# microsoft/tutel

Measured on NVIDIA H100. Metric: moe_layer_fwd_bwd_tokens_per_sec, higher is better.
Workload: dtype bf16; 1 GPU; model=helloworld moe_layer top-2 8-expert ffn(relu) model_dim=4096 hidden=14336, global_batch=16, seq_len=512, parallelism=ep1 (8 local experts/GPU), a2a_ffn_overlap_degree=1, cuda_graph=True, launches_per_graph_replay=15

## Files before the change

### csrc/gemm_sm90.cu

```cuda
#include "gemm_sm90.h"

#include <cuda.h>
#include <cuda_bf16.h>
#include <cuda_fp16.h>

#include <cstdio>
#include <cstdlib>
#include <mutex>

#include "ptx.cuh"

namespace tb {

struct GemmArgs {
  int M, N, K, G;
  int b_group_div;
  int tiles_m, tiles_n;
  long long num_tiles;

  void* d;
  long long ldd, d_group_stride;
  const unsigned long long* d_ptr_table;
  int out_dtype;

// ... 30 lines not shown
namespace {

constexpr int kThreads = 384;
constexpr int kSwizzleBytes = 128;
constexpr int kSmemLimit = 232448;

template <int BN_>
struct Cfg {
  static constexpr int BM = 128;
  static constexpr int BN = BN_;
  static constexpr bool WIDE = BN_ == 256;
  static constexpr int A_BYTES = BM * kSwizzleBytes;
  static constexpr int B_BYTES = BN * kSwizzleBytes;
  static constexpr int STAGE_BYTES = A_BYTES + B_BYTES;
  static constexpr int EPI_COLS = 128;
  static constexpr int PASSES = BN / EPI_COLS;
  static constexpr int EPI_PITCH = EPI_COLS + 8;
  static constexpr int EPI_WARP_BYTES = 16 * EPI_PITCH * 4;
  static constexpr int EPI_BYTES = 8 * EPI_WARP_BYTES;
  static constexpr int BAR_BYTES = 512;
  static constexpr int STAGES = WIDE ? 3 : 4;
  static constexpr int MAXNREG = WIDE ? 168 : 144;
  static constexpr int CONSUMER_REGS = WIDE ? 232 : 192;
  static constexpr int SMEM_BYTES = STAGES * STAGE_BYTES + 1024 + BAR_BYTES + EPI_BYTES;
  static_assert(WIDE || SMEM_BYTES + 2 * 1024 <= 228 * 1024, "no room for the push kernel");
  static_assert(SMEM_BYTES <= kSmemLimit, "");
  static_assert(128 * 40 + 256 * CONSUMER_REGS <= 65536 && 384 * MAXNREG <= 65536, "register budget");
};

struct TileCoord {
  int g, m_blk, n_blk;
};

template <int kBand>
__device__ __forceinline__ TileCoord decode_tile(long long t, int tiles_m, int tiles_n) {
  const int per_group = tiles_m * tiles_n;
  TileCoord c;
  c.g = static_cast<int>(t / per_group);
  int r = static_cast<int>(t - static_cast<long long>(c.g) * per_group);
// ... 10 lines not shown
__device__ __forceinline__ int rotate_group(int g, int rot, int mod) {
  if (mod > 1) {
    const int base = (g / mod) * mod;
    return base + (g - base + rot) % mod;
  }
  if (mod < -1) {
    const int m = -mod;
    const int base = (g / m) * m;
    return base + (rot + m - (g - base)) % m;
  }
  return g;
}

__device__ __forceinline__ float gelu_erf(float x) { return 0.5f * x * (1.0f + erff(x * 0.70710678118654752f)); }
__device__ __forceinline__ float silu(float x) { return __fdividef(x, 1.0f + __expf(-x)); }

__device__ __forceinline__ void unpack8(const uint4& u, bool is_bf16, float* f) {
  const uint32_t w[4] = {u.x, u.y, u.z, u.w};
#pragma unroll
  for (int i = 0; i < 4; ++i) {
    if (is_bf16) {
      f[2 * i] = __uint_as_float(w[i] << 16);
      f[2 * i + 1] = __uint_as_float(w[i] & 0xFFFF0000u);
    } else {
      const __half2 h = *reinterpret_cast<const __half2*>(&w[i]);
      const float2 t = __half22float2(h);
      f[2 * i] = t.x;
      f[2 * i + 1] = t.y;
    }
  }
// ... 23 lines not shown
    for (int i = 0; i < 4; ++i) {
      if constexpr (BF16) {
        f[q * 8 + 2 * i] = __uint_as_float(w[i] << 16);
        f[q * 8 + 2 * i + 1] = __uint_as_float(w[i] & 0xFFFF0000u);
      } else {
        const float2 t = __half22float2(*reinterpret_cast<const __half2*>(&w[i]));
        f[q * 8 + 2 * i] = t.x;
        f[q * 8 + 2 * i + 1] = t.y;
      }
    }
  }
}
__device__ __forceinline__ void unpack32(const uint4* p, float* f, bool is_bf16) {
  if (is_bf16) unpack32_t<true>(p, f); else unpack32_t<false>(p, f);
}

__device__ __forceinline__ float fast_sigmoid(float x) { return __fdividef(1.0f, 1.0f + __expf(-x)); }

template <int ACT>
__device__ __forceinline__ void glu_fwd_seg(const float* g, const float* u, float* o) {
#pragma unroll
  for (int j = 0; j < 32; ++j) {
    float a;
    if constexpr (ACT == ACT_RELU) a = fmaxf(g[j], 0.0f);
    else if constexpr (ACT == ACT_GELU) a = gelu_erf(g[j]);
    else a = g[j] * fast_sigmoid(g[j]);
    o[j] = a * u[j];
  }
}
template <int ACT>
__device__ __forceinline__ void glu_bwd_seg(const float* r, const float* g, float* u, float* o) {
#pragma unroll
// ... 5 lines not shown
      da = g[j] > 0.0f ? 1.0f : 0.0f;
    } else if constexpr (ACT == ACT_GELU) {
      const float cdf = 0.5f * (1.0f + erff(g[j] * 0.70710678118654752f));
      a = g[j] * cdf;
      da = cdf + g[j] * 0.3989422804014327f * __expf(-0.5f * g[j] * g[j]);
    } else {
      const float sg = fast_sigmoid(g[j]);
      a = g[j] * sg;
      da = sg * (1.0f + g[j] * (1.0f - sg));
    }
    o[j] = dh * u[j] * da;
    u[j] = dh * a;
  }
}

template <int BN_, bool A_MN, bool B_MN, int DT>
__global__ void __maxnreg__(Cfg<BN_>::MAXNREG)
gemm_sm90_kernel(const __grid_constant__ CUtensorMap tmA, const __grid_constant__ CUtensorMap tmB,
                 const __grid_constant__ CUtensorMap tmB2, const GemmArgs args) {
  using C = Cfg<BN_>;
  constexpr int BN = C::BN;
  extern __shared__ uint8_t smem_raw[];

  const int warp = __shfl_sync(0xffffffffu, static_cast<int>(threadIdx.x >> 5), 0);
  const int lane = threadIdx.x & 31;

  const uint32_t smem_base = (ptx::smem_u32(smem_raw) + 1023u) & ~1023u;
  constexpr int stages = C::STAGES;
  const uint32_t bar_base = smem_base + static_cast<uint32_t>(stages) * C::STAGE_BYTES;
  auto smem_a = [&](int s) { return smem_base + s * C::STAGE_BYTES; };
  auto smem_b = [&](int s) { return smem_base + s * C::STAGE_BYTES + C::A_BYTES; };
  auto full_bar = [&](int s) { return bar_base + 8u * s; };
  auto empty_bar = [&](int s) { return bar_base + 64u + 8u * s; };
  const uint32_t epi_base = bar_base + C::BAR_BYTES;
  float* epi_ptr = reinterpret_cast<float*>(smem_raw + (epi_base - ptx::smem_u32(smem_raw)));

  if (warp == 0 && ptx::elect_one()) {
    ptx::prefetch_tensormap(&tmA);
    ptx::prefetch_tensormap(&tmB);
    if (args.dual) ptx::prefetch_tensormap(&tmB2);
  }
  if (warp == 1 && lane == 0) {
    for (int s = 0; s < stages; ++s) {
      ptx::mbar_init(full_bar(s), 1);
      ptx::mbar_init(empty_bar(s), 2);
    }
    ptx::fence_mbar_init();
  }
  __syncthreads();

  constexpr int kEltBytes = (DT == DT_E4M3 || DT == DT_E5M2) ? 1 : 2;
  static_assert(kEltBytes == 2 || (!A_MN && !B_MN), "8-bit operands are K-major only");
  const int num_kb = (args.K * kEltBytes + kSwizzleBytes - 1) / kSwizzleBytes;
  constexpr int bk_elems = kSwizzleBytes / kEltBytes;
  const long long tile_step = gridDim.x;
  const long long tile_first = blockIdx.x;
  constexpr int kBand = 16;
  const bool dual = !C::WIDE && args.dual != 0;
  const int tile_n = dual ? BN / 2 : BN;

  if (warp < 4) {
    ptx::setmaxnreg_dec<40>();
    if (warp == 0) {
      int s = 0;
      uint32_t ph = 0;
      int seen_group = -1;
      unsigned long long seen_mask = 0ull;
      for (long long t = tile_first; t < args.num_tiles; t += tile_step) {
        TileCoord tc = decode_tile<kBand>(t, args.tiles_m, args.tiles_n);
        tc.g = rotate_group(tc.g, args.group_rot, args.group_mod);
        if (args.row_counts != nullptr && tc.m_blk * C::BM >= args.row_counts[tc.g]) continue;
        const int m0 = tc.m_blk * C::BM;
        const int n0 = tc.n_blk * BN;
        const int gb = tc.g / args.b_group_div;
        if (args.wait_flags != nullptr) {
          if (tc.g != seen_group) { seen_group = tc.g; seen_mask = 0ull; }
          const int f0 = (tc.m_blk * C::BM) / args.wait_rows_per_flag;
          const int f1 = (min(tc.m_blk * C::BM + C::BM, args.M) - 1) / args.wait_rows_per_flag;
          unsigned long long need = 0ull;
          for (int f = f0; f <= f1; ++f) need |= 1ull << (f & 63);
// ... 33 lines not shown
            } else {
              const int nb0 = tc.n_blk * (BN / 2);
              if constexpr (!B_MN) {
                ptx::tma_load_3d(smem_b(s), &tmB, fb, k0, nb0, gb);
                ptx::tma_load_3d(smem_b(s) + (BN / 2) * kSwizzleBytes, &tmB2, fb, k0, nb0, gb);
              } else {
                constexpr int half_chunks = (BN / 2) / chunk_elems;
                for (int c = 0; c < 2 * half_chunks; ++c)
                  ptx::tma_load_3d(smem_b(s) + c * chunk_bytes, c < half_chunks ? &tmB : &tmB2, fb,
                                   nb0 + (c % half_chunks) * chunk_elems, k0, gb);
              }
            }
          }
          __syncwarp();
          if (++s == stages) { s = 0; ph ^= 1u; }
        }
      }
    }
  } else {
    ptx::setmaxnreg_inc<C::CONSUMER_REGS>();
    const int cw = warp - 4;
    const int wg = cw >> 2;
    const bool wg_leader = (threadIdx.x & 127) == 0;
    int s = 0;
    uint32_t ph = 0;
    constexpr uint32_t kMnChunkBytes = 64u * kSwizzleBytes;
    constexpr uint32_t kMnKStep = 16u * kSwizzleBytes;
    constexpr uint32_t a_lbo = A_MN ? kMnChunkBytes : 16u;
    constexpr uint32_t b_lbo = B_MN ? kMnChunkBytes : 16u;
    constexpr uint32_t a_kstep = (A_MN ? kMnKStep : 32u) >> 4;
    constexpr uint32_t b_kstep = (B_MN ? kMnKStep : 32u) >> 4;
// ... 2 lines not shown
    const uint32_t b_lo0 = ((smem_b(0) >> 4) & 0x3FFFu) | ((b_lbo >> 4) << 16);

    const bool out16 = (args.out_dtype != DT_FP32);
    const bool out_bf16 = (args.out_dtype == DT_BF16);
    const bool glu = !C::WIDE && (args.epilogue == EPI_GLU || args.epilogue == EPI_GLU_BWD);
    float* epi_warp = epi_ptr + cw * 16 * C::EPI_PITCH;
    const float* epi_row = epi_warp + (lane & 15) * C::EPI_PITCH;
    const int col_half = (lane >> 4) * 32;
    auto load_acc = [&](int col, float* v) {
#pragma unroll
      for (int q = 0; q < 8; ++q) {
        const float4 t4 = *reinterpret_cast<const float4*>(epi_row + col + q * 4);
        v[q * 4] = t4.x; v[q * 4 + 1] = t4.y; v[q * 4 + 2] = t4.z; v[q * 4 + 3] = t4.w;
      }
    };

    for (long long t = tile_first; t < args.num_tiles; t += tile_step) {
      TileCoord tc = decode_tile<kBand>(t, args.tiles_m, args.tiles_n);
      tc.g = rotate_group(tc.g, args.group_rot, args.group_mod);
      int m_valid = args.M;
      if (args.row_counts != nullptr) {
        m_valid = min(args.M, args.row_counts[tc.g]);
        if (tc.m_blk * C::BM >= m_valid) continue;
      }
      float acc[BN / 2];
      int prev_s = 0;
      for (int kb = 0; kb < num_kb; ++kb) {
        ptx::mbar_wait_quiet(full_bar(s), ph);
        const uint32_t a_lo = a_lo0 + static_cast<uint32_t>(s) * (C::STAGE_BYTES >> 4);
        const uint32_t b_lo = b_lo0 + static_cast<uint32_t>(s) * (C::STAGE_BYTES >> 4);
        ptx::wgmma_fence();
#pragma unroll
        for (int k = 0; k < 4; ++k) {
          const uint64_t ad = (static_cast<uint64_t>(desc_hi) << 32) | (a_lo + k * a_kstep);
          const uint64_t bd = (static_cast<uint64_t>(desc_hi) << 32) | (b_lo + k * b_kstep);
          if constexpr (BN == 256) ptx::wgmma_m64n256<DT, A_MN, B_MN>(acc, ad, bd, (kb | k) != 0);
          else ptx::wgmma_m64n128<DT, A_MN, B_MN>(acc, ad, bd, (kb | k) != 0);
        }
        ptx::wgmma_commit();
        if (kb > 0) {
          ptx::wgmma_wait<1>();
          if (wg_leader) ptx::mbar_arrive(empty_bar(prev_s));
        }
        prev_s = s;
        if (++s == stages) { s = 0; ph ^= 1u; }
      }
      ptx::wgmma_wait<0>();
      if (wg_leader) ptx::mbar_arrive(empty_bar(prev_s));

#pragma unroll
      for (int pass = 0; pass < C::PASSES; ++pass) {
      {
        const int fr = lane >> 2, fc = (lane & 3) * 2;
#pragma unroll
        for (int jj = 0; jj < C::EPI_COLS / 8; ++jj) {
          const int j = pass * (C::EPI_COLS / 8) + jj;
          *reinterpret_cast<float2*>(epi_warp + fr * C::EPI_PITCH + jj * 8 + fc) = make_float2(acc[4 * j], acc[4 * j + 1]);
          *reinterpret_cast<float2*>(epi_warp + (fr + 8) * C::EPI_PITCH + jj * 8 + fc) = make_float2(acc[4 * j + 2], acc[4 * j + 3]);
        }
      }
      __syncwarp();

      const int m = tc.m_blk * C::BM + cw * 16 + (lane & 15);
      const bool row_ok = m < m_valid;
      const int gb = tc.g / args.b_group_div;
      uint8_t* d_base = (args.d_ptr_table != nullptr)
                            ? reinterpret_cast<uint8_t*>(args.d_ptr_table[tc.g])
                            : reinterpret_cast<uint8_t*>(args.d) +
                                  static_cast<long long>(tc.g) * args.d_group_stride * (out16 ? 2 : 4);
      uint8_t* d_row = d_base + static_cast<long long>(m) * args.ldd * (out16 ? 2 : 4);
      const uint8_t* aux_row = nullptr;
      if (args.aux != nullptr)
        aux_row = reinterpret_cast<const uint8_t*>(args.aux) +
// ... 78 lines not shown
              for (int j = 0; j < 32; ++j) dh[j] *= (sb != nullptr && j < ncols) ? sa * sb[j] : sa;
            }
            load_seg16(aux_row, n, ncols, g);
            load_seg16(aux2_row, n, ncols, u);
            if (args.act == ACT_RELU) glu_bwd_seg<ACT_RELU>(dh, g, u, o);
            else if (args.act == ACT_GELU) glu_bwd_seg<ACT_GELU>(dh, g, u, o);
            else glu_bwd_seg<ACT_SILU>(dh, g, u, o);
            store_seg(d_row, n, ncols, o);
            store_seg(d2_row, n, ncols, u);
          }
        }
      } else {
#pragma unroll 1
      for (int c = 0; c < C::EPI_COLS / 64; ++c) {
        const int col = c * 64 + col_half;
        const int n = tc.n_blk * BN + pass * C::EPI_COLS + col;
        float v[32];
        load_acc(col, v);
        const int ncols = min(32, args.N - n);
        if (args.scale_a != nullptr || args.scale_b != nullptr) {
          const float sa = (args.scale_a != nullptr && row_ok)
                               ? args.scale_a[static_cast<long long>(tc.g) * args.scale_a_group_stride + m] : 1.0f;
          const float* sb = args.scale_b != nullptr ? args.scale_b + static_cast<long long>(gb) * args.scale_b_group_stride + n : nullptr;
#pragma unroll
          for (int j = 0; j < 32; ++j) v[j] *= (sb != nullptr && j < ncols) ? sa * sb[j] : sa;
        }

        if (args.epilogue == EPI_NONE) {
          if (args.alpha != 1.0f) {
#pragma unroll
            for (int j = 0; j < 32; ++j) v[j] *= args.alpha;
          }
        } else if (args.epilogue == EPI_RELU_BWD || args.epilogue == EPI_ADD || args.epilogue == EPI_ACT_BWD) {
          float f[32];
          load_seg16(aux_row, n, ncols, f);
          if (args.epilogue == EPI_RELU_BWD) {
#pragma unroll
            for (int j = 0; j < 32; ++j) v[j] = f[j] > 0.0f ? v[j] : 0.0f;
          } else if (args.epilogue == EPI_ADD) {
#pragma unroll
            for (int j = 0; j < 32; ++j) v[j] += f[j];
          } else if (args.act == ACT_GELU) {
#pragma unroll
            for (int j = 0; j < 32; ++j) {
              const float cdf = 0.5f * (1.0f + erff(f[j] * 0.70710678118654752f));
              v[j] *= cdf + f[j] * 0.3989422804014327f * __expf(-0.5f * f[j] * f[j]);
            }
          } else if (args.act == ACT_SILU) {
#pragma unroll
            for (int j = 0; j < 32; ++j) {
              const float sg = fast_sigmoid(f[j]);
              v[j] *= sg * (1.0f + f[j] * (1.0f - sg));
            }
          } else {
#pragma unroll
            for (int j = 0; j < 32; ++j) v[j] = f[j] > 0.0f ? v[j] : 0.0f;
          }
        } else {
          if (bias_g != nullptr) {
#pragma unroll
            for (int q = 0; q < 4; ++q) {
              if (q * 8 < ncols) {
                float f[8];
                if (args.bias_is_fp32) {
                  const float4 b0 = *reinterpret_cast<const float4*>(bias_g + (n + q * 8) * 4);
                  const float4 b1 = *reinterpret_cast<const float4*>(bias_g + (n + q * 8 + 4) * 4);
                  f[0] = b0.x; f[1] = b0.y; f[2] = b0.z; f[3] = b0.w;
                  f[4] = b1.x; f[5] = b1.y; f[6] = b1.z; f[7] = b1.w;
                } else {
                  unpack8(*reinterpret_cast<const uint4*>(bias_g + (n + q * 8) * 2), args.bias_is_bf16 != 0, f);
                }
// ... 32 lines not shown
              const float recv = __shfl_xor_sync(0xffffffffu, send, off);
              s[i] = (upper ? s[i + 2 * off] : s[i]) + recv;
            }
          }
          const int cc = 2 * (lane & 15);
          float* cs = args.colsum + static_cast<long long>(gb) * args.colsum_group_stride + n + cc;
          if (cc < ncols) {
            atomicAdd(cs, s[0]);
            atomicAdd(cs + 1, s[1]);
          }
        }
        store_seg(d_row, n, ncols, v);
      }
      }
      __syncwarp();
      }
      if (args.signal_ptr_table != nullptr) {
        asm volatile("bar.sync 1, 256;" ::: "memory");
        if (cw == 0 && lane == 0) {
          ptx::fence_acq_rel_sys();
          ptx::red_add_release_sys(reinterpret_cast<uint32_t*>(args.signal_ptr_table[tc.g]), 1u);
        }
      }
    }
  }
}

using EncodeTiledFn = CUresult (*)(CUtensorMap*, CUtensorMapDataType, cuuint32_t, void*, const cuuint64_t*,
                                   const cuuint64_t*, const cuuint32_t*, const cuuint32_t*, CUtensorMapInterleave,
                                   CUtensorMapSwizzle, CUtensorMapL2promotion, CUtensorMapFloatOOBfill);

EncodeTiledFn get_encode_fn() {
  static EncodeTiledFn fn = nullptr;
  static std::once_flag once;
  std::call_once(once, [] {
    void* p = nullptr;
    cudaDriverEntryPointQueryResult q;
    if (cudaGetDriverEntryPoint("cuTensorMapEncodeTiled", &p, cudaEnableDefault, &q) == cudaSuccess &&
// ... 26 lines not shown
  } else {
    dims[0] = static_cast<cuuint64_t>(rows_mn); dims[1] = static_cast<cuuint64_t>(k);
    box[0] = row_elems; box[1] = row_elems;
  }
  dims[2] = static_cast<cuuint64_t>(groups);
  box[2] = 1;
  strides[0] = static_cast<cuuint64_t>(ld) * eb;
  strides[1] = static_cast<cuuint64_t>(groups > 1 ? group_stride : (mn_major ? k : rows_mn) * ld) * eb;
  if (strides[1] == 0) strides[1] = strides[0];
  CUresult r = enc(map, dt, 3, const_cast<void*>(base), dims, strides, box, estr, CU_TENSOR_MAP_INTERLEAVE_NONE,
                   CU_TENSOR_MAP_SWIZZLE_128B, CU_TENSOR_MAP_L2_PROMOTION_L2_256B, CU_TENSOR_MAP_FLOAT_OOB_FILL_NONE);
  if (r != CUDA_SUCCESS) { *why = "cuTensorMapEncodeTiled failed"; return false; }
  return true;
}

template <int BN, bool A_MN, bool B_MN, int DT>
cudaError_t launch_inst(const CUtensorMap& ta, const CUtensorMap& tb_, const CUtensorMap& tb2, const GemmArgs& args,
                        int grid, cudaStream_t stream) {
  auto* kern = gemm_sm90_kernel<BN, A_MN, B_MN, DT>;
  static bool configured = false;
  if (!configured) {
    cudaError_t e = cudaFuncSetAttribute(kern, cudaFuncAttributeMaxDynamicSharedMemorySize, Cfg<BN>::SMEM_BYTES);
    if (e != cudaSuccess) return e;
    configured = true;
  }
  kern<<<grid, kThreads, Cfg<BN>::SMEM_BYTES, stream>>>(ta, tb_, tb2, args);
  return cudaGetLastError();
}

}

cudaError_t gemm_sm90_launch(const GemmProblem& p, cudaStream_t stream, const char** why_out) {
  const char* why_local = nullptr;
  const char** why = why_out ? why_out : &why_local;
  *why = nullptr;
  if (p.M <= 0 || p.N <= 0 || p.K <= 0 || p.G <= 0) return cudaSuccess;
  const int eb = (p.in_dtype == DT_E4M3 || p.in_dtype == DT_E5M2) ? 1 : 2;
  if (p.N % 8 != 0) { *why = "N must be a multiple of 8"; return cudaErrorInvalidValue; }
  const int ob = p.out_dtype == DT_FP32 ? 4 : 2;
  if ((reinterpret_cast<uintptr_t>(p.d) & 15) || ((p.ldd * ob) & 15) || ((p.d_group_stride * ob) & 15)) {
    *why = "output base/stride must be 16-byte aligned";
// ... 13 lines not shown
    *why = "EPI_GLU_BWD needs aux, aux2, d2 and a 16-bit output";
    return cudaErrorInvalidValue;
  }
  if ((p.epilogue == EPI_GLU || p.epilogue == EPI_GLU_BWD) && p.d_ptr_table != nullptr) { *why = "GLU epilogues write local outputs only"; return cudaErrorInvalidValue; }
  const bool uses_aux = p.epilogue == EPI_RELU_BWD || p.epilogue == EPI_ADD || p.epilogue == EPI_GLU_BWD || p.epilogue == EPI_ACT_BWD;
  if (uses_aux && (p.aux == nullptr || p.out_dtype == DT_FP32 ||
                   ((reinterpret_cast<uintptr_t>(p.aux) | reinterpret_cast<uintptr_t>(p.aux2)) & 15) || ((p.ld_aux * 2) & 15) ||
                   ((p.aux_group_stride * 2) & 15))) {
    *why = "this epilogue needs a 16-byte aligned 16-bit aux operand";
    return cudaErrorInvalidValue;
  }
  if (p.cta_group < 0 || p.cta_group > 2) { *why = "cta_group must be 0, 1 or 2"; return cudaErrorInvalidValue; }
  if (p.block_n != 0 && p.block_n != 128 && p.block_n != 256) { *why = "block_n must be 0, 128 or 256"; return cudaErrorInvalidValue; }

  const bool wide = p.block_n != 128 && p.wait_flags == nullptr && p.signal_ptr_table == nullptr && p.d_ptr_table == nullptr &&
                    p.epilogue != EPI_GLU && p.epilogue != EPI_GLU_BWD;
  constexpr int bm = 128;
  const int bn = wide ? 256 : 128;
  GemmArgs a{};
  a.M = p.M; a.N = p.N; a.K = p.K; a.G = p.G;
  a.b_group_div = p.b_group_div > 0 ? p.b_group_div : 1;
  a.tiles_m = (p.M + bm - 1) / bm;
  a.tiles_n = dual ? (p.N + bn / 2 - 1) / (bn / 2) : (p.N + bn - 1) / bn;
  a.num_tiles = static_cast<long long>(a.tiles_m) * a.tiles_n * p.G;
  a.d = p.d; a.ldd = p.ldd; a.d_group_stride = p.d_group_stride; a.d_ptr_table = p.d_ptr_table;
  a.out_dtype = p.out_dtype;
  a.epilogue = p.epilogue; a.alpha = p.alpha;
  a.bias = p.bias; a.bias_group_stride = p.bias_group_stride; a.bias_is_fp32 = 0;
  a.bias_is_bf16 = (eb == 2) ? (p.in_dtype == DT_BF16) : (p.out_dtype == DT_BF16);
  a.aux = p.aux; a.ld_aux = p.ld_aux; a.aux_group_stride = p.aux_group_stride;
  a.aux2 = p.aux2; a.d2 = p.d2; a.d3 = p.d3; a.dual = dual ? 1 : 0; a.act = p.act; a.scale_b2 = p.scale_b2;
// ... 4 lines not shown
  a.wait_flags = p.wait_flags; a.wait_rows_per_flag = p.wait_rows_per_flag > 0 ? p.wait_rows_per_flag : bm;
  a.wait_flags_per_group = p.wait_flags_per_group; a.wait_target = p.wait_target;
  a.signal_ptr_table = p.signal_ptr_table;
  a.group_rot = p.group_rot; a.group_mod = p.group_mod;

  CUtensorMap ta, tb_;
  const int gB = (p.G + a.b_group_div - 1) / a.b_group_div;
  if (!make_operand_map(&ta, p.a, p.in_dtype, p.a_mn_major, p.M, p.K, p.lda, p.a_group_stride, p.G, bm, why))
    return cudaErrorInvalidValue;
  const int b_box = dual ? bn / 2 : bn;
  if (!make_operand_map(&tb_, p.b, p.in_dtype, p.b_mn_major, p.N, p.K, p.ldb, p.b_group_stride, gB, b_box, why))
    return cudaErrorInvalidValue;
  CUtensorMap tb2 = tb_;
  if (dual && !make_operand_map(&tb2, p.b2, p.in_dtype, p.b_mn_major, p.N, p.K, p.ldb, p.b_group_stride, gB, b_box, why))
    return cudaErrorInvalidValue;

  const int grid = static_cast<int>(a.num_tiles < sms ? a.num_tiles : sms);

  if (eb == 1) {
    if (p.a_mn_major || p.b_mn_major) { *why = "fp8 operands must be K-major"; return cudaErrorInvalidValue; }
    const bool xact = p.epilogue == EPI_BIAS_GELU || p.epilogue == EPI_BIAS_SILU || p.epilogue == EPI_ACT_BWD;
    if (xact) { *why = "GELU / SiLU epilogues need 16-bit operands"; return cudaErrorInvalidValue; }
    if (wide) {
      if (p.in_dtype == DT_E4M3) return launch_inst<256, false, false, DT_E4M3>(ta, tb_, tb2, a, grid, stream);
      return launch_inst<256, false, false, DT_E5M2>(ta, tb_, tb2, a, grid, stream);
    }
    if (p.in_dtype == DT_E4M3) return launch_inst<128, false, false, DT_E4M3>(ta, tb_, tb2, a, grid, stream);
    return launch_inst<128, false, false, DT_E5M2>(ta, tb_, tb2, a, grid, stream);
  }
#define TB_SWITCH_MAJOR(BNv, DTv)                                                                                  \
  do {                                                                                                             \
    if (!p.a_mn_major && !p.b_mn_major) return launch_inst<BNv, false, false, DTv>(ta, tb_, tb2, a, grid, stream);   \
    if (!p.a_mn_major && p.b_mn_major) return launch_inst<BNv, false, true, DTv>(ta, tb_, tb2, a, grid, stream);     \
    if (p.a_mn_major && !p.b_mn_major) return launch_inst<BNv, true, false, DTv>(ta, tb_, tb2, a, grid, stream);     \
    return launch_inst<BNv, true, true, DTv>(ta, tb_, tb2, a, grid, stream);                                        \
  } while (0)
  if (p.in_dtype == DT_BF16) { if (wide) TB_SWITCH_MAJOR(256, DT_BF16); TB_SWITCH_MAJOR(128, DT_BF16); }
  if (p.in_dtype == DT_FP16) { if (wide) TB_SWITCH_MAJOR(256, DT_FP16); TB_SWITCH_MAJOR(128, DT_FP16); }
#undef TB_SWITCH_MAJOR
  *why = "unsupported operand dtype";
  return cudaErrorInvalidValue;
}

cudaError_t set_spin_timeout_gemm(unsigned long long ns) {
  return cudaMemcpyToSymbol(tb_spin_timeout_ns, &ns, sizeof(ns));
}

}
```

### csrc/ptx.cuh

```cuda
#pragma once
#include <cstdint>
#include <cstdio>
#include <cuda.h>
#include <cuda_runtime.h>

#ifndef TB_SPIN_TIMEOUT_NS
#define TB_SPIN_TIMEOUT_NS 300000000000ull
#endif

static __constant__ unsigned long long tb_spin_timeout_ns = TB_SPIN_TIMEOUT_NS;

namespace ptx {

__device__ __forceinline__ uint32_t smem_u32(const void* p) {
  return static_cast<uint32_t>(__cvta_generic_to_shared(p));
}

__device__ __forceinline__ uint64_t globaltimer_ns() {
  uint64_t t;
  asm volatile("mov.u64 %0, %%globaltimer;" : "=l"(t));
  return t;
}

__device__ __forceinline__ uint32_t elect_one() {
// ... 163 lines not shown
                                            int c2) {
  asm volatile(
      "cp.async.bulk.tensor.3d.shared::cluster.global.mbarrier::complete_tx::bytes"
      " [%0], [%1, {%3, %4, %5}], [%2];" ::"r"(smem_dst),
      "l"(tmap), "r"(bar), "r"(c0), "r"(c1), "r"(c2)
      : "memory");
}
__device__ __forceinline__ void prefetch_l2_bulk(const void* gptr, uint32_t bytes) {
  asm volatile("cp.async.bulk.prefetch.L2.global [%0], %1;" ::"l"(gptr), "r"(bytes) : "memory");
}

__device__ __forceinline__ void tma_store_3d(const void* tmap, uint32_t smem_src, int c0, int c1, int c2) {
  asm volatile("cp.async.bulk.tensor.3d.global.shared::cta.bulk_group [%0, {%2, %3, %4}], [%1];" ::"l"(tmap),
               "r"(smem_src), "r"(c0), "r"(c1), "r"(c2)
               : "memory");
}

__device__ __forceinline__ void wgmma_fence() { asm volatile("wgmma.fence.sync.aligned;" ::: "memory"); }
__device__ __forceinline__ void wgmma_commit() { asm volatile("wgmma.commit_group.sync.aligned;" ::: "memory"); }
template <int N>
__device__ __forceinline__ void wgmma_wait() { asm volatile("wgmma.wait_group.sync.aligned %0;" ::"n"(N) : "memory"); }

enum WgmmaType : int { WG_BF16 = 0, WG_FP16 = 1, WG_E4M3 = 3, WG_E5M2 = 4 };

#define TB_ACC8(d, o) "+f"(d[o]), "+f"(d[o + 1]), "+f"(d[o + 2]), "+f"(d[o + 3]), "+f"(d[o + 4]), "+f"(d[o + 5]), "+f"(d[o + 6]), "+f"(d[o + 7])
#define TB_ACC64(d) TB_ACC8(d, 0), TB_ACC8(d, 8), TB_ACC8(d, 16), TB_ACC8(d, 24), TB_ACC8(d, 32), TB_ACC8(d, 40), TB_ACC8(d, 48), TB_ACC8(d, 56)
#define TB_D64 "{%0, %1, %2, %3, %4, %5, %6, %7, %8, %9, %10, %11, %12, %13, %14, %15, %16, %17, %18, %19, %20, %21, %22, %23, %24, %25, %26, %27, %28, %29, %30, %31, %32, %33, %34, %35, %36, %37, %38, %39, %40, %41, %42, %43, %44, %45, %46, %47, %48, %49, %50, %51, %52, %53, %54, %55, %56, %57, %58, %59, %60, %61, %62, %63}"
#define TB_WGMMA16(TYPES)                                                                                       \
  asm volatile("{\n\t.reg .pred p;\n\tsetp.ne.b32 p, %66, 0;\n\t"                                               \
               "wgmma.mma_async.sync.aligned.m64n128k16.f32." TYPES " " TB_D64 ", %64, %65, p, 1, 1, %67, %68;\n\t}\n" \
// ... 63 lines not shown
```

Baseline: 409,400 tokens/s.

## Stage wide-tile epilogue through swizzled smem with TMA store and TMA-prefetched aux

For the BN=256 path, the epilogue no longer passes through the per-warp fp32 staging buffer. Accumulators are now packed to 16-bit into a 128B-swizzled shared output tile and written back with TMA bulk stores. The producer warp TMA-loads the aux tensor (for relu/act backward and add epilogues) into the same tile during the mainloop, and an out_empty mbarrier guards reuse across tiles. Column sums use a shuffle reduction plus shared-memory atomics. This aims to overlap the output store and aux reads with the next tile's MMA. In exchange it adds shared memory use and extra barrier handshakes, and it excludes fp32 outputs from the wide path.

Measured after the change: 440,100 tokens/s (median of 6 runs). 1.08x the previous value.

```diff
diff --git a/csrc/gemm_sm90.cu b/csrc/gemm_sm90.cu
--- a/csrc/gemm_sm90.cu
+++ b/csrc/gemm_sm90.cu
@@ -68,15 +68,18 @@
   static constexpr int B_BYTES = BN * kSwizzleBytes;
   static constexpr int STAGE_BYTES = A_BYTES + B_BYTES;
   static constexpr int EPI_COLS = 128;
-  static constexpr int PASSES = BN / EPI_COLS;
   static constexpr int EPI_PITCH = EPI_COLS + 8;
   static constexpr int EPI_WARP_BYTES = 16 * EPI_PITCH * 4;
-  static constexpr int EPI_BYTES = 8 * EPI_WARP_BYTES;
+  static constexpr int EPI_BYTES = WIDE ? 0 : 8 * EPI_WARP_BYTES;
+  static constexpr int OUT_BOX_BYTES = BM * kSwizzleBytes;
+  static constexpr int OUT_TILE_BYTES = WIDE ? BM * BN * 2 : 0;
+  static constexpr int COLSUM_BYTES = WIDE ? 2 * BN * 4 : 0;
   static constexpr int BAR_BYTES = 512;
   static constexpr int STAGES = WIDE ? 3 : 4;
   static constexpr int MAXNREG = WIDE ? 168 : 144;
   static constexpr int CONSUMER_REGS = WIDE ? 232 : 192;
-  static constexpr int SMEM_BYTES = STAGES * STAGE_BYTES + 1024 + BAR_BYTES + EPI_BYTES;
+  static constexpr int SMEM_BYTES = STAGES * STAGE_BYTES + 1024 + OUT_TILE_BYTES + BAR_BYTES + EPI_BYTES + COLSUM_BYTES;
+  static_assert((STAGES * STAGE_BYTES) % 1024 == 0, "the output tile must stay 1024B aligned for the 128B swizzle");
   static_assert(WIDE || SMEM_BYTES + 2 * 1024 <= 228 * 1024, "no room for the push kernel");
   static_assert(SMEM_BYTES <= kSmemLimit, "");
   static_assert(128 * 40 + 256 * CONSUMER_REGS <= 65536 && 384 * MAXNREG <= 65536, "register budget");
@@ -117,6 +120,25 @@
 
 __device__ __forceinline__ float gelu_erf(float x) { return 0.5f * x * (1.0f + erff(x * 0.70710678118654752f)); }
 __device__ __forceinline__ float silu(float x) { return __fdividef(x, 1.0f + __expf(-x)); }
+__device__ __forceinline__ float fast_sigmoid(float x) { return __fdividef(1.0f, 1.0f + __expf(-x)); }
+__device__ __forceinline__ float relu_bwd(float v, float x) { return x > 0.0f ? v : 0.0f; }
+__device__ __forceinline__ float gelu_bwd(float v, float x) {
+  const float cdf = 0.5f * (1.0f + erff(x * 0.70710678118654752f));
+  return v * (cdf + x * 0.3989422804014327f * __expf(-0.5f * x * x));
+}
+__device__ __forceinline__ float silu_bwd(float v, float x) {
+  const float sg = fast_sigmoid(x);
+  return v * (sg * (1.0f + x * (1.0f - sg)));
+}
+__device__ __forceinline__ uint32_t pack2(float a, float b, bool bf16) {
+  const __nv_bfloat162 hb = __floats2bfloat162_rn(a, b);
+  const __half2 hh = __floats2half2_rn(a, b);
+  return bf16 ? *reinterpret_cast<const uint32_t*>(&hb) : *reinterpret_cast<const uint32_t*>(&hh);
+}
+__device__ __forceinline__ float2 unpack2(uint32_t w, bool bf16) {
+  const float2 h = __half22float2(*reinterpret_cast<const __half2*>(&w));
+  return bf16 ? make_float2(__uint_as_float(w << 16), __uint_as_float(w & 0xFFFF0000u)) : h;
+}
 
 __device__ __forceinline__ void unpack8(const uint4& u, bool is_bf16, float* f) {
   const uint32_t w[4] = {u.x, u.y, u.z, u.w};
@@ -170,8 +192,6 @@
 __device__ __forceinline__ void unpack32(const uint4* p, float* f, bool is_bf16) {
   if (is_bf16) unpack32_t<true>(p, f); else unpack32_t<false>(p, f);
 }
-
-__device__ __forceinline__ float fast_sigmoid(float x) { return __fdividef(1.0f, 1.0f + __expf(-x)); }
 
 template <int ACT>
 __device__ __forceinline__ void glu_fwd_seg(const float* g, const float* u, float* o) {
@@ -207,10 +227,141 @@
   }
 }
 
+enum WideMain : int { WM_NONE, WM_BIAS, WM_RELU_BWD, WM_ADD, WM_GELU_BWD, WM_SILU_BWD };
+
+__device__ __forceinline__ uint32_t out_tile_off(int j, int swz) {
+  return static_cast<uint32_t>((j >> 3) * (128 * kSwizzleBytes) + (((j & 7) ^ swz) << 4));
+}
+
+__device__ __forceinline__ void wide_scale(float (&acc)[128], float sa0, float sa1, const float* sb, int n_lane, int N) {
+#pragma unroll
+  for (int j = 0; j < 32; ++j) {
+    const int n = n_lane + 8 * j;
+    if (sb != nullptr && n < N) {
+      const float2 s = *reinterpret_cast<const float2*>(sb + n);
+      acc[4 * j] *= sa0 * s.x; acc[4 * j + 1] *= sa0 * s.y;
+      acc[4 * j + 2] *= sa1 * s.x; acc[4 * j + 3] *= sa1 * s.y;
+    } else {
+      acc[4 * j] *= sa0; acc[4 * j + 1] *= sa0;
+      acc[4 * j + 2] *= sa1; acc[4 * j + 3] *= sa1;
+    }
+  }
+}
+
+template <int WM>
+__device__ __forceinline__ void wide_main(float (&acc)[128], const uint8_t* row0, int swz, const uint8_t* bias_g,
+                                          bool bias_f32, bool bias_bf16, int n_lane, int N, bool out_bf16, float alpha) {
+#pragma unroll
+  for (int j = 0; j < 32; ++j) {
+    if constexpr (WM == WM_NONE) {
+#pragma unroll
+      for (int c = 0; c < 4; ++c) acc[4 * j + c] *= alpha;
+    } else if constexpr (WM == WM_BIAS) {
+      const int n = n_lane + 8 * j;
+      float2 b = make_float2(0.0f, 0.0f);
+      if (n < N)
+        b = bias_f32 ? *reinterpret_cast<const float2*>(bias_g + n * 4)
+                     : unpack2(*reinterpret_cast<const uint32_t*>(bias_g + n * 2), bias_bf16);
+      acc[4 * j] += b.x; acc[4 * j + 1] += b.y;
+      acc[4 * j + 2] += b.x; acc[4 * j + 3] += b.y;
+    } else {
+      const uint32_t o = out_tile_off(j, swz);
+#pragma unroll
+      for (int h = 0; h < 2; ++h) {
+        const float2 f = unpack2(*reinterpret_cast<const uint32_t*>(row0 + h * 8 * kSwizzleBytes + o), out_bf16);
+        float& v0 = acc[4 * j + 2 * h];
+        float& v1 = acc[4 * j + 2 * h + 1];
+        if constexpr (WM == WM_RELU_BWD) { v0 = relu_bwd(v0, f.x); v1 = relu_bwd(v1, f.y); }
+        else if constexpr (WM == WM_ADD) { v0 += f.x; v1 += f.y; }
+        else if constexpr (WM == WM_GELU_BWD) { v0 = gelu_bwd(v0, f.x); v1 = gelu_bwd(v1, f.y); }
+        else { v0 = silu_bwd(v0, f.x); v1 = silu_bwd(v1, f.y); }
+      }
+    }
+  }
+}
+
+template <int ACT>
+__device__ __forceinline__ void wide_act(float (&acc)[128]) {
+#pragma unroll
+  for (int i = 0; i < 128; ++i) {
+    if constexpr (ACT == ACT_RELU) acc[i] = fmaxf(acc[i], 0.0f);
+    else if constexpr (ACT == ACT_GELU) acc[i] = gelu_erf(acc[i]);
+    else acc[i] = silu(acc[i]);
+  }
+}
+
+__device__ __forceinline__ void wide_stage(const float (&acc)[128], uint8_t* row0, int swz, bool out_bf16) {
+#pragma unroll
+  for (int j = 0; j < 32; ++j) {
+    const uint32_t o = out_tile_off(j, swz);
+    *reinterpret_cast<uint32_t*>(row0 + o) = pack2(acc[4 * j], acc[4 * j + 1], out_bf16);
+    *reinterpret_cast<uint32_t*>(row0 + 8 * kSwizzleBytes + o) = pack2(acc[4 * j + 2], acc[4 * j + 3], out_bf16);
+  }
+}
+
+__device__ __forceinline__ void wide_colsum(const float (&acc)[128], bool ok0, bool ok1, int lane, float* colrow) {
+  float s[64];
+#pragma unroll
+  for (int j = 0; j < 32; ++j) {
+#pragma unroll
+    for (int c = 0; c < 2; ++c) s[2 * j + c] = (ok0 ? acc[4 * j + c] : 0.0f) + (ok1 ? acc[4 * j + 2 + c] : 0.0f);
+  }
+#pragma unroll
+  for (int off = 16; off >= 4; off >>= 1) {
+    const bool upper = (lane & off) != 0;
+#pragma unroll
+    for (int i = 0; i < 2 * off; ++i) {
+      const float send = upper ? s[i] : s[i + 2 * off];
+      const float recv = __shfl_xor_sync(0xffffffffu, send, off);
+      s[i] = (upper ? s[i + 2 * off] : s[i]) + recv;
+    }
+  }
+  float* base = colrow + 32 * (lane >> 2) + 2 * (lane & 3);
+#pragma unroll
+  for (int i = 0; i < 8; ++i) atomicAdd(base + 8 * (i >> 1) + (i & 1), s[i]);
+}
+
+struct OutTileStore {
+  const uint8_t* tile;
+  uint32_t tile_smem;
+  int m0, n0, m_valid, N, g;
+  long long group_stride, ld;
+  bool straddle;
+  int ct;
+  bool writer;
+};
+__device__ __forceinline__ void flush_out_tile(const OutTileStore& s, const CUtensorMap* map, uint8_t* dst, bool wait_read) {
+  constexpr int kChunks = 256 / 8;
+  ptx::fence_proxy_async_smem();
+  ptx::named_bar_sync(1, 256);
+  if (s.straddle) {
+    for (int i = s.ct; i < 128 * kChunks; i += 256) {
+      const int r = i / kChunks, ch = i % kChunks;
+      const int m = s.m0 + r, n = s.n0 + ch * 8;
+      if (m < s.m_valid && n < s.N) {
+        const uint4 v = *reinterpret_cast<const uint4*>(s.tile + (ch >> 3) * (128 * kSwizzleBytes) + r * kSwizzleBytes +
+                                                        (((ch & 7) ^ (r & 7)) << 4));
+        *reinterpret_cast<uint4*>(dst + (static_cast<long long>(s.g) * s.group_stride + static_cast<long long>(m) * s.ld + n) * 2) = v;
+      }
+    }
+    ptx::named_bar_sync(1, 256);
+    return;
+  }
+  if (s.writer) {
+    for (int b = 0; b < 4; ++b)
+      if (s.n0 + 64 * b < s.N) ptx::tma_store_3d(map, s.tile_smem + b * (128 * kSwizzleBytes), s.n0 + 64 * b, s.m0, s.g);
+    ptx::bulk_commit_group();
+    if (wait_read) ptx::bulk_wait_group_read<0>();
+  }
+  if (wait_read) ptx::named_bar_sync(1, 256);
+}
+
 template <int BN_, bool A_MN, bool B_MN, int DT>
 __global__ void __maxnreg__(Cfg<BN_>::MAXNREG)
 gemm_sm90_kernel(const __grid_constant__ CUtensorMap tmA, const __grid_constant__ CUtensorMap tmB,
-                 const __grid_constant__ CUtensorMap tmB2, const GemmArgs args) {
+                 const __grid_constant__ CUtensorMap tmB2, const __grid_constant__ CUtensorMap tmD,
+                 const __grid_constant__ CUtensorMap tmAux, const __grid_constant__ CUtensorMap tmD2,
+                 const GemmArgs args) {
   using C = Cfg<BN_>;
   constexpr int BN = C::BN;
   extern __shared__ uint8_t smem_raw[];
@@ -220,25 +371,38 @@
 
   const uint32_t smem_base = (ptx::smem_u32(smem_raw) + 1023u) & ~1023u;
   constexpr int stages = C::STAGES;
-  const uint32_t bar_base = smem_base + static_cast<uint32_t>(stages) * C::STAGE_BYTES;
+  const uint32_t out_base = smem_base + static_cast<uint32_t>(stages) * C::STAGE_BYTES;
+  const uint32_t bar_base = out_base + C::OUT_TILE_BYTES;
   auto smem_a = [&](int s) { return smem_base + s * C::STAGE_BYTES; };
   auto smem_b = [&](int s) { return smem_base + s * C::STAGE_BYTES + C::A_BYTES; };
   auto full_bar = [&](int s) { return bar_base + 8u * s; };
   auto empty_bar = [&](int s) { return bar_base + 64u + 8u * s; };
+  const uint32_t aux_full = bar_base + 128u;
+  const uint32_t out_empty = bar_base + 136u;
   const uint32_t epi_base = bar_base + C::BAR_BYTES;
   float* epi_ptr = reinterpret_cast<float*>(smem_raw + (epi_base - ptx::smem_u32(smem_raw)));
+  uint8_t* out_tile = smem_raw + (out_base - ptx::smem_u32(smem_raw));
+  float* colsum_rows = epi_ptr;
+  const bool aux_tma = C::WIDE && (args.epilogue == EPI_RELU_BWD || args.epilogue == EPI_ADD || args.epilogue == EPI_ACT_BWD);
 
   if (warp == 0 && ptx::elect_one()) {
     ptx::prefetch_tensormap(&tmA);
     ptx::prefetch_tensormap(&tmB);
     if (args.dual) ptx::prefetch_tensormap(&tmB2);
+    if (C::WIDE) ptx::prefetch_tensormap(&tmD);
+    if (aux_tma) ptx::prefetch_tensormap(&tmAux);
   }
   if (warp == 1 && lane == 0) {
     for (int s = 0; s < stages; ++s) {
       ptx::mbar_init(full_bar(s), 1);
       ptx::mbar_init(empty_bar(s), 2);
     }
+    ptx::mbar_init(aux_full, 1);
+    ptx::mbar_init(out_empty, 1);
     ptx::fence_mbar_init();
+  }
+  if constexpr (C::WIDE) {
+    for (int i = threadIdx.x; i < 2 * BN; i += kThreads) colsum_rows[i] = 0.0f;
   }
   __syncthreads();
 
@@ -251,12 +415,14 @@
   constexpr int kBand = 16;
   const bool dual = !C::WIDE && args.dual != 0;
   const int tile_n = dual ? BN / 2 : BN;
+  const int kb_out_free = min(2, num_kb - 1);
 
   if (warp < 4) {
     ptx::setmaxnreg_dec<40>();
     if (warp == 0) {
       int s = 0;
       uint32_t ph = 0;
+      uint32_t it = 0;
       int seen_group = -1;
       unsigned long long seen_mask = 0ull;
       for (long long t = tile_first; t < args.num_tiles; t += tile_step) {
@@ -320,7 +486,17 @@
           }
           __syncwarp();
           if (++s == stages) { s = 0; ph ^= 1u; }
-        }
+          if (aux_tma && kb == kb_out_free) {
+            ptx::mbar_wait_quiet(out_empty, (it & 1u) ^ 1u);
+            if (ptx::elect_one()) {
+              ptx::mbar_expect_tx(aux_full, C::OUT_TILE_BYTES);
+              for (int b = 0; b < BN / 64; ++b)
+                ptx::tma_load_3d(out_base + b * C::OUT_BOX_BYTES, &tmAux, aux_full, n0 + 64 * b, m0, tc.g);
+            }
+            __syncwarp();
+          }
+        }
+        ++it;
       }
     }
   } else {
@@ -353,6 +529,17 @@
         v[q * 4] = t4.x; v[q * 4 + 1] = t4.y; v[q * 4 + 2] = t4.z; v[q * 4 + 3] = t4.w;
       }
     };
+    const int ct = threadIdx.x - 128;
+    const bool out_writer = ct == 0;
+    const int r0 = cw * 16 + (lane >> 2);
+    const int swz = lane >> 2;
+    uint8_t* row0 = out_tile + r0 * kSwizzleBytes + (lane & 3) * 4;
+    const int wmain = args.epilogue == EPI_NONE ? WM_NONE
+                    : args.epilogue == EPI_ADD ? WM_ADD
+                    : args.epilogue == EPI_RELU_BWD ? WM_RELU_BWD
+                    : args.epilogue == EPI_ACT_BWD ? (args.act == ACT_GELU ? WM_GELU_BWD : args.act == ACT_SILU ? WM_SILU_BWD : WM_RELU_BWD)
+                    : WM_BIAS;
+    uint32_t it = 0;
 
     for (long long t = tile_first; t < args.num_tiles; t += tile_step) {
       TileCoord tc = decode_tile<kBand>(t, args.tiles_m, args.tiles_n);
@@ -363,6 +550,10 @@
         if (tc.m_blk * C::BM >= m_valid) continue;
       }
       float acc[BN / 2];
+      if constexpr (C::WIDE) {
+#pragma unroll
+        for (int i = 0; i < BN / 2; ++i) acc[i] = 0.0f;
+      }
       int prev_s = 0;
       for (int kb = 0; kb < num_kb; ++kb) {
         ptx::mbar_wait_quiet(full_bar(s), ph);
@@ -377,6 +568,13 @@
           else ptx::wgmma_m64n128<DT, A_MN, B_MN>(acc, ad, bd, (kb | k) != 0);
         }
         ptx::wgmma_commit();
+        if constexpr (C::WIDE) {
+          if (out_writer && it > 0 && kb == kb_out_free) {
+            ptx::bulk_wait_group_read<0>();
+            ptx::mbar_arrive(out_empty);
+          }
+          __syncwarp();
+        }
         if (kb > 0) {
           ptx::wgmma_wait<1>();
           if (wg_leader) ptx::mbar_arrive(empty_bar(prev_s));
@@ -387,15 +585,77 @@
       ptx::wgmma_wait<0>();
       if (wg_leader) ptx::mbar_arrive(empty_bar(prev_s));
 
-#pragma unroll
-      for (int pass = 0; pass < C::PASSES; ++pass) {
+      if constexpr (C::WIDE) {
+        const int m0 = tc.m_blk * C::BM, n0 = tc.n_blk * BN;
+        const int gb = tc.g / args.b_group_div;
+        const bool ok0 = m0 + r0 < m_valid, ok1 = m0 + r0 + 8 < m_valid;
+        const int n_lane = n0 + 2 * (lane & 3);
+        const bool straddle = m0 + C::BM > m_valid && m_valid < args.M;
+        if (args.scale_a != nullptr || args.scale_b != nullptr) {
+          const float* sa = args.scale_a != nullptr ? args.scale_a + static_cast<long long>(tc.g) * args.scale_a_group_stride + m0 + r0 : nullptr;
+          const float sa0 = (sa != nullptr && ok0) ? sa[0] : 1.0f;
+          const float sa1 = (sa != nullptr && ok1) ? sa[8] : 1.0f;
+          const float* sb = args.scale_b != nullptr ? args.scale_b + static_cast<long long>(gb) * args.scale_b_group_stride : nullptr;
+          wide_scale(acc, sa0, sa1, sb, n_lane, args.N);
+        }
+        const uint8_t* bias_g = nullptr;
+        if (args.bias != nullptr)
+          bias_g = reinterpret_cast<const uint8_t*>(args.bias) +
+                   static_cast<long long>(gb) * args.bias_group_stride * (args.bias_is_fp32 ? 4 : 2);
+        const uint32_t out_free_parity = (it & 1u) ^ 1u;
+
+        const OutTileStore st{out_tile, out_base, m0, n0, m_valid, args.N, tc.g, args.d_group_stride, args.ldd, straddle, ct,
+                              out_writer};
+
+        if (wmain == WM_BIAS) {
+          if (bias_g != nullptr)
+            wide_main<WM_BIAS>(acc, row0, swz, bias_g, args.bias_is_fp32 != 0, args.bias_is_bf16 != 0, n_lane, args.N, out_bf16, 1.0f);
+          if (args.d2 != nullptr && (args.epilogue == EPI_BIAS_GELU || args.epilogue == EPI_BIAS_SILU)) {
+            ptx::mbar_wait_quiet(out_empty, out_free_parity);
+            wide_stage(acc, row0, swz, out_bf16);
+            flush_out_tile(st, &tmD2, reinterpret_cast<uint8_t*>(args.d2), true);
+          }
+          if (args.epilogue == EPI_BIAS_RELU) wide_act<ACT_RELU>(acc);
+          else if (args.epilogue == EPI_BIAS_GELU) wide_act<ACT_GELU>(acc);
+          else if (args.epilogue == EPI_BIAS_SILU) wide_act<ACT_SILU>(acc);
+        } else if (wmain == WM_NONE) {
+          if (args.alpha != 1.0f) wide_main<WM_NONE>(acc, row0, swz, nullptr, false, false, n_lane, args.N, out_bf16, args.alpha);
+        } else {
+          ptx::mbar_wait_quiet(aux_full, it & 1u);
+          if (wmain == WM_RELU_BWD) wide_main<WM_RELU_BWD>(acc, row0, swz, nullptr, false, false, n_lane, args.N, out_bf16, 1.0f);
+          else if (wmain == WM_ADD) wide_main<WM_ADD>(acc, row0, swz, nullptr, false, false, n_lane, args.N, out_bf16, 1.0f);
+          else if (wmain == WM_GELU_BWD) wide_main<WM_GELU_BWD>(acc, row0, swz, nullptr, false, false, n_lane, args.N, out_bf16, 1.0f);
+          else wide_main<WM_SILU_BWD>(acc, row0, swz, nullptr, false, false, n_lane, args.N, out_bf16, 1.0f);
+        }
+        if (!aux_tma) ptx::mbar_wait_quiet(out_empty, out_free_parity);
+        wide_stage(acc, row0, swz, out_bf16);
+        float* colrow = colsum_rows + (it & 1u) * BN;
+        if (args.colsum != nullptr) wide_colsum(acc, ok0, ok1, lane, colrow);
+        flush_out_tile(st, &tmD, reinterpret_cast<uint8_t*>(args.d), false);
+        if (args.colsum != nullptr && ct < BN / 4) {
+          float4* src = reinterpret_cast<float4*>(colrow) + ct;
+          const float4 v = *src;
+          *src = make_float4(0.0f, 0.0f, 0.0f, 0.0f);
+          const int n = n0 + 4 * ct;
+          if (n < args.N) {
+            float* cs = args.colsum + static_cast<long long>(gb) * args.colsum_group_stride + n;
+            if ((reinterpret_cast<uintptr_t>(cs) & 15) == 0) {
+              ptx::red_add_v4_f32(cs, v.x, v.y, v.z, v.w);
+            } else {
+              atomicAdd(cs, v.x); atomicAdd(cs + 1, v.y); atomicAdd(cs + 2, v.z); atomicAdd(cs + 3, v.w);
+            }
+          }
+        }
+        ++it;
+        continue;
+      }
+
       {
         const int fr = lane >> 2, fc = (lane & 3) * 2;
 #pragma unroll
-        for (int jj = 0; jj < C::EPI_COLS / 8; ++jj) {
-          const int j = pass * (C::EPI_COLS / 8) + jj;
-          *reinterpret_cast<float2*>(epi_warp + fr * C::EPI_PITCH + jj * 8 + fc) = make_float2(acc[4 * j], acc[4 * j + 1]);
-          *reinterpret_cast<float2*>(epi_warp + (fr + 8) * C::EPI_PITCH + jj * 8 + fc) = make_float2(acc[4 * j + 2], acc[4 * j + 3]);
+        for (int j = 0; j < C::EPI_COLS / 8; ++j) {
+          *reinterpret_cast<float2*>(epi_warp + fr * C::EPI_PITCH + j * 8 + fc) = make_float2(acc[4 * j], acc[4 * j + 1]);
+          *reinterpret_cast<float2*>(epi_warp + (fr + 8) * C::EPI_PITCH + j * 8 + fc) = make_float2(acc[4 * j + 2], acc[4 * j + 3]);
         }
       }
       __syncwarp();
@@ -504,7 +764,7 @@
 #pragma unroll 1
       for (int c = 0; c < C::EPI_COLS / 64; ++c) {
         const int col = c * 64 + col_half;
-        const int n = tc.n_blk * BN + pass * C::EPI_COLS + col;
+        const int n = tc.n_blk * BN + col;
         float v[32];
         load_acc(col, v);
         const int ncols = min(32, args.N - n);
@@ -526,25 +786,19 @@
           load_seg16(aux_row, n, ncols, f);
           if (args.epilogue == EPI_RELU_BWD) {
 #pragma unroll
-            for (int j = 0; j < 32; ++j) v[j] = f[j] > 0.0f ? v[j] : 0.0f;
+            for (int j = 0; j < 32; ++j) v[j] = relu_bwd(v[j], f[j]);
           } else if (args.epilogue == EPI_ADD) {
 #pragma unroll
             for (int j = 0; j < 32; ++j) v[j] += f[j];
           } else if (args.act == ACT_GELU) {
 #pragma unroll
-            for (int j = 0; j < 32; ++j) {
-              const float cdf = 0.5f * (1.0f + erff(f[j] * 0.70710678118654752f));
-              v[j] *= cdf + f[j] * 0.3989422804014327f * __expf(-0.5f * f[j] * f[j]);
-            }
+            for (int j = 0; j < 32; ++j) v[j] = gelu_bwd(v[j], f[j]);
           } else if (args.act == ACT_SILU) {
 #pragma unroll
-            for (int j = 0; j < 32; ++j) {
-              const float sg = fast_sigmoid(f[j]);
-              v[j] *= sg * (1.0f + f[j] * (1.0f - sg));
-            }
+            for (int j = 0; j < 32; ++j) v[j] = silu_bwd(v[j], f[j]);
           } else {
 #pragma unroll
-            for (int j = 0; j < 32; ++j) v[j] = f[j] > 0.0f ? v[j] : 0.0f;
+            for (int j = 0; j < 32; ++j) v[j] = relu_bwd(v[j], f[j]);
           }
         } else {
           if (bias_g != nullptr) {
@@ -607,7 +861,6 @@
       }
       }
       __syncwarp();
-      }
       if (args.signal_ptr_table != nullptr) {
         asm volatile("bar.sync 1, 256;" ::: "memory");
         if (cw == 0 && lane == 0) {
@@ -615,6 +868,9 @@
           ptx::red_add_release_sys(reinterpret_cast<uint32_t*>(args.signal_ptr_table[tc.g]), 1u);
         }
       }
+    }
+    if constexpr (C::WIDE) {
+      if (out_writer) ptx::bulk_wait_group<0>();
     }
   }
 }
@@ -671,9 +927,31 @@
   return true;
 }
 
+bool make_tile_map(CUtensorMap* map, const void* base, int dtype, long long rows, long long cols, long long ld,
+                   long long group_stride, int groups, const char** why) {
+  EncodeTiledFn enc = get_encode_fn();
+  if (enc == nullptr) { *why = "cuTensorMapEncodeTiled unavailable"; return false; }
+  if ((reinterpret_cast<uintptr_t>(base) & 15) || ((ld * 2) & 15) || ((group_stride * 2) & 15)) {
+    *why = "output / aux base and strides must be 16-byte aligned";
+    return false;
+  }
+  const cuuint64_t dims[3] = {static_cast<cuuint64_t>(cols), static_cast<cuuint64_t>(rows), static_cast<cuuint64_t>(groups)};
+  cuuint64_t strides[2] = {static_cast<cuuint64_t>(ld) * 2,
+                           static_cast<cuuint64_t>(groups > 1 ? group_stride : rows * ld) * 2};
+  if (strides[1] == 0) strides[1] = strides[0];
+  const cuuint32_t box[3] = {64, 128, 1};
+  const cuuint32_t estr[3] = {1, 1, 1};
+  CUresult r = enc(map, dtype == DT_BF16 ? CU_TENSOR_MAP_DATA_TYPE_BFLOAT16 : CU_TENSOR_MAP_DATA_TYPE_FLOAT16, 3,
+                   const_cast<void*>(base), dims, strides, box, estr, CU_TENSOR_MAP_INTERLEAVE_NONE,
+                   CU_TENSOR_MAP_SWIZZLE_128B, CU_TENSOR_MAP_L2_PROMOTION_L2_256B, CU_TENSOR_MAP_FLOAT_OOB_FILL_NONE);
+  if (r != CUDA_SUCCESS) { *why = "cuTensorMapEncodeTiled failed"; return false; }
+  return true;
+}
+
 template <int BN, bool A_MN, bool B_MN, int DT>
-cudaError_t launch_inst(const CUtensorMap& ta, const CUtensorMap& tb_, const CUtensorMap& tb2, const GemmArgs& args,
-                        int grid, cudaStream_t stream) {
+cudaError_t launch_inst(const CUtensorMap& ta, const CUtensorMap& tb_, const CUtensorMap& tb2, const CUtensorMap& td,
+                        const CUtensorMap& taux, const CUtensorMap& td2, const GemmArgs& args, int grid,
+                        cudaStream_t stream) {
   auto* kern = gemm_sm90_kernel<BN, A_MN, B_MN, DT>;
   static bool configured = false;
   if (!configured) {
@@ -681,7 +959,7 @@
     if (e != cudaSuccess) return e;
     configured = true;
   }
-  kern<<<grid, kThreads, Cfg<BN>::SMEM_BYTES, stream>>>(ta, tb_, tb2, args);
+  kern<<<grid, kThreads, Cfg<BN>::SMEM_BYTES, stream>>>(ta, tb_, tb2, td, taux, td2, args);
   return cudaGetLastError();
 }
 
@@ -725,7 +1003,7 @@
   if (p.block_n != 0 && p.block_n != 128 && p.block_n != 256) { *why = "block_n must be 0, 128 or 256"; return cudaErrorInvalidValue; }
 
   const bool wide = p.block_n != 128 && p.wait_flags == nullptr && p.signal_ptr_table == nullptr && p.d_ptr_table == nullptr &&
-                    p.epilogue != EPI_GLU && p.epilogue != EPI_GLU_BWD;
+                    p.epilogue != EPI_GLU && p.epilogue != EPI_GLU_BWD && p.out_dtype != DT_FP32;
   constexpr int bm = 128;
   const int bn = wide ? 256 : 128;
   GemmArgs a{};
@@ -760,6 +1038,15 @@
   CUtensorMap tb2 = tb_;
   if (dual && !make_operand_map(&tb2, p.b2, p.in_dtype, p.b_mn_major, p.N, p.K, p.ldb, p.b_group_stride, gB, b_box, why))
     return cudaErrorInvalidValue;
+  CUtensorMap td = tb_, taux = tb_, td2 = tb_;
+  if (wide) {
+    if (!make_tile_map(&td, p.d, p.out_dtype, p.M, p.N, p.ldd, p.d_group_stride, p.G, why)) return cudaErrorInvalidValue;
+    if (uses_aux && !make_tile_map(&taux, p.aux, p.out_dtype, p.M, p.N, p.ld_aux, p.aux_group_stride, p.G, why))
+      return cudaErrorInvalidValue;
+    if (p.d2 != nullptr && (p.epilogue == EPI_BIAS_GELU || p.epilogue == EPI_BIAS_SILU) &&
+        !make_tile_map(&td2, p.d2, p.out_dtype, p.M, p.N, p.ldd, p.d_group_stride, p.G, why))
+      return cudaErrorInvalidValue;
+  }
 
   const int grid = static_cast<int>(a.num_tiles < sms ? a.num_tiles : sms);
 
@@ -768,18 +1055,18 @@
     const bool xact = p.epilogue == EPI_BIAS_GELU || p.epilogue == EPI_BIAS_SILU || p.epilogue == EPI_ACT_BWD;
     if (xact) { *why = "GELU / SiLU epilogues need 16-bit operands"; return cudaErrorInvalidValue; }
     if (wide) {
-      if (p.in_dtype == DT_E4M3) return launch_inst<256, false, false, DT_E4M3>(ta, tb_, tb2, a, grid, stream);
-      return launch_inst<256, false, false, DT_E5M2>(ta, tb_, tb2, a, grid, stream);
-    }
-    if (p.in_dtype == DT_E4M3) return launch_inst<128, false, false, DT_E4M3>(ta, tb_, tb2, a, grid, stream);
-    return launch_inst<128, false, false, DT_E5M2>(ta, tb_, tb2, a, grid, stream);
+      if (p.in_dtype == DT_E4M3) return launch_inst<256, false, false, DT_E4M3>(ta, tb_, tb2, td, taux, td2, a, grid, stream);
+      return launch_inst<256, false, false, DT_E5M2>(ta, tb_, tb2, td, taux, td2, a, grid, stream);
+    }
+    if (p.in_dtype == DT_E4M3) return launch_inst<128, false, false, DT_E4M3>(ta, tb_, tb2, td, taux, td2, a, grid, stream);
+    return launch_inst<128, false, false, DT_E5M2>(ta, tb_, tb2, td, taux, td2, a, grid, stream);
   }
 #define TB_SWITCH_MAJOR(BNv, DTv)                                                                                  \
   do {                                                                                                             \
-    if (!p.a_mn_major && !p.b_mn_major) return launch_inst<BNv, false, false, DTv>(ta, tb_, tb2, a, grid, stream);   \
-    if (!p.a_mn_major && p.b_mn_major) return launch_inst<BNv, false, true, DTv>(ta, tb_, tb2, a, grid, stream);     \
-    if (p.a_mn_major && !p.b_mn_major) return launch_inst<BNv, true, false, DTv>(ta, tb_, tb2, a, grid, stream);     \
-    return launch_inst<BNv, true, true, DTv>(ta, tb_, tb2, a, grid, stream);                                        \
+    if (!p.a_mn_major && !p.b_mn_major) return launch_inst<BNv, false, false, DTv>(ta, tb_, tb2, td, taux, td2, a, grid, stream);   \
+    if (!p.a_mn_major && p.b_mn_major) return launch_inst<BNv, false, true, DTv>(ta, tb_, tb2, td, taux, td2, a, grid, stream);     \
+    if (p.a_mn_major && !p.b_mn_major) return launch_inst<BNv, true, false, DTv>(ta, tb_, tb2, td, taux, td2, a, grid, stream);     \
+    return launch_inst<BNv, true, true, DTv>(ta, tb_, tb2, td, taux, td2, a, grid, stream);                                        \
   } while (0)
   if (p.in_dtype == DT_BF16) { if (wide) TB_SWITCH_MAJOR(256, DT_BF16); TB_SWITCH_MAJOR(128, DT_BF16); }
   if (p.in_dtype == DT_FP16) { if (wide) TB_SWITCH_MAJOR(256, DT_FP16); TB_SWITCH_MAJOR(128, DT_FP16); }
diff --git a/csrc/ptx.cuh b/csrc/ptx.cuh
--- a/csrc/ptx.cuh
+++ b/csrc/ptx.cuh
@@ -201,6 +201,19 @@
   asm volatile("cp.async.bulk.tensor.3d.global.shared::cta.bulk_group [%0, {%2, %3, %4}], [%1];" ::"l"(tmap),
                "r"(smem_src), "r"(c0), "r"(c1), "r"(c2)
                : "memory");
+}
+__device__ __forceinline__ void bulk_commit_group() { asm volatile("cp.async.bulk.commit_group;" ::: "memory"); }
+template <int N>
+__device__ __forceinline__ void bulk_wait_group_read() { asm volatile("cp.async.bulk.wait_group.read %0;" ::"n"(N) : "memory"); }
+template <int N>
+__device__ __forceinline__ void bulk_wait_group() { asm volatile("cp.async.bulk.wait_group %0;" ::"n"(N) : "memory"); }
+
+__device__ __forceinline__ void named_bar_sync(int id, int count) {
+  asm volatile("bar.sync %0, %1;" ::"r"(id), "r"(count) : "memory");
+}
+
+__device__ __forceinline__ void red_add_v4_f32(float* p, float a, float b, float c, float d) {
+  asm volatile("red.global.add.v4.f32 [%0], {%1, %2, %3, %4};" ::"l"(p), "f"(a), "f"(b), "f"(c), "f"(d) : "memory");
 }
 
 __device__ __forceinline__ void wgmma_fence() { asm volatile("wgmma.fence.sync.aligned;" ::: "memory"); }
```
